# naver-ai/egtr

Hardware: AMD Instinct MI355X
Metric: images/sec end-to-end SGG, 600x1000 input, N=200 queries (higher is better)
Workload: dtype f32; 1 GPU; VG inference: ResNet-50, N=200, 6 enc/6 dec, 150 classes, 50 predicates, 600x1000, bs=1/GPU fp32 (BASELINE configs[1]); hip_graph=True, gemm_tuning=True, miopen_find=True, parallelism=replicas x1 (independent images, no collective)

## Files before the change

egtr_amd/csrc/ffn_x6.hip:

```cpp
#include <hip/hip_runtime.h>
#include <stdint.h>

#include "common.h"
#include "x6_common.h"
#include "xs_format.h"

namespace {
using namespace x6;

constexpr int kD = 256;
constexpr int kRows = 64;
constexpr int kKS = kD / 16;
constexpr int kFrag = xs::kFragBytes;
constexpr int kPanel = 2 * kKS * 2 * kFrag;
constexpr int kHbuf = 2 * 4 * 3 * kFrag;
constexpr int kStage = 24 * kFrag;
constexpr int kLds = kPanel + kHbuf + 3 * kStage;
static_assert(kLds == 160 * 1024, "the whole LDS of a CU");
constexpr int NL = 6;
typedef float f32x8 __attribute__((ext_vector_type(8)));

struct FfnArgs {
  const float* x;
  const float* res;
  const char* w1;
  const float* b1;
  const char* w2;
  const float* b2;
  const float* gamma;
  const float* beta;
  const float* pos;
  float* out;
  float* out_pos;
  int M, ldx, ldr, F, pos_rows;
  float eps;
  const char* wp;
  const float* bp;
  const float* gamma1;
  const float* beta1;
  float eps1;
};

__device__ __forceinline__ int swz(int x, int ks) { return x ^ (ks & 15) ^ ((x >> 5) << 2); }

__device__ __forceinline__ void build_panel(const float* __restrict__ x, int ldx, int M, int r0, int tid, int lane,
                                            char* panel, char* lo0, char* lo1) {
  float4 v[16];
#pragma unroll
  for (int it = 0; it < 16; ++it) {
    const int row = min(r0 + it * 4 + (tid >> 6), M - 1);
    v[it] = *reinterpret_cast<const float4*>(x + (size_t)row * ldx + 4 * lane);
  }
#pragma unroll
  for (int it = 0; it < 16; ++it) {
    const int row = it * 4 + (tid >> 6), rb = row >> 5, r = row & 31;
    const int ks = lane >> 2, off = (swz(r + 32 * ((lane >> 1) & 1), ks) << 4) + (lane & 1) * 8;
    const xs::Split3 s0 = xs::split3_fast(v[it].x), s1 = xs::split3_fast(v[it].y), s2 = xs::split3_fast(v[it].z),
                     s3 = xs::split3_fast(v[it].w);
    char* p = panel + ((rb * kKS + ks) * 2) * kFrag + off;
    *reinterpret_cast<uint2*>(p) = make_uint2(xs::pack_hi16(s0.hi, s1.hi), xs::pack_hi16(s2.hi, s3.hi));
    *reinterpret_cast<uint2*>(p + kFrag) = make_uint2(xs::pack_hi16(s0.mid, s1.mid), xs::pack_hi16(s2.mid, s3.mid));
    char* q = (rb == 0 ? lo0 : lo1) + ks * kFrag + off;
    *reinterpret_cast<uint2*>(q) = make_uint2(xs::pack_hi16(s0.lo, s1.lo), xs::pack_hi16(s2.lo, s3.lo));
  }
}

template <bool USE_RES_OF, class ResFn>
__device__ __forceinline__ void final_epilogue(const f32x16 (&acc2)[4], const FfnArgs& A, int r0, int wave, int lane,
                                               float* red, ResFn&& res_of) {
  const int wm = wave >> 1, wn = wave & 1, li = lane & 31, hf = lane >> 5;
  const int row = r0 + wm * 32 + li;
  float4 y[4][4];
#pragma unroll
  for (int t = 0; t < 4; ++t)
#pragma unroll
    for (int q = 0; q < 4; ++q) {
      const int col = (4 * wn + t) * 32 + 8 * q + 4 * hf;
      const float4 b = A.b2 != nullptr ? *reinterpret_cast<const float4*>(A.b2 + col) : make_float4(0.f, 0.f, 0.f, 0.f);
      y[t][q] = make_float4(acc2[t][4 * q + 0] + b.x, acc2[t][4 * q + 1] + b.y, acc2[t][4 * q + 2] + b.z,
                            acc2[t][4 * q + 3] + b.w);
    }
  if (A.gamma != nullptr) {
    const float* xr = A.res + (size_t)min(row, A.M - 1) * A.ldr;
#pragma unroll
    for (int t = 0; t < 4; ++t)
#pragma unroll
      for (int q = 0; q < 4; ++q) {
        float4 r;
        if constexpr (USE_RES_OF) r = res_of(t, q);
        else r = *reinterpret_cast<const float4*>(xr + (4 * wn + t) * 32 + 8 * q + 4 * hf);
        y[t][q].x += r.x; y[t][q].y += r.y; y[t][q].z += r.z; y[t][q].w += r.w;
      }
    __syncthreads();
    float sum = 0.f;
#pragma unroll
    for (int t = 0; t < 4; ++t)
#pragma unroll
      for (int q = 0; q < 4; ++q) sum += (y[t][q].x + y[t][q].y) + (y[t][q].z + y[t][q].w);
    sum += __shfl_xor(sum, 32);
    if (hf == 0) red[wave * 32 + li] = sum;
    __syncthreads();
    const float mean = (sum + red[(wave ^ 1) * 32 + li]) * (1.f / kD);
    float sq = 0.f;
#pragma unroll
    for (int t = 0; t < 4; ++t)
#pragma unroll
      for (int q = 0; q < 4; ++q) {
        y[t][q].x -= mean; y[t][q].y -= mean; y[t][q].z -= mean; y[t][q].w -= mean;
        sq += (y[t][q].x * y[t][q].x + y[t][q].y * y[t][q].y) + (y[t][q].z * y[t][q].z + y[t][q].w * y[t][q].w);
      }
    sq += __shfl_xor(sq, 32);
    if (hf == 0) red[128 + wave * 32 + li] = sq;
    __syncthreads();
    const float rstd = rsqrtf((sq + red[128 + (wave ^ 1) * 32 + li]) * (1.f / kD) + A.eps);
    const float* pr = A.out_pos != nullptr ? A.pos + (size_t)(min(row, A.M - 1) % A.pos_rows) * kD : nullptr;
#pragma unroll
    for (int t = 0; t < 4; ++t)
#pragma unroll
      for (int q = 0; q < 4; ++q) {
        const int col = (4 * wn + t) * 32 + 8 * q + 4 * hf;
        const float4 g = *reinterpret_cast<const float4*>(A.gamma + col), b = *reinterpret_cast<const float4*>(A.beta + col);
        y[t][q] = make_float4(y[t][q].x * rstd * g.x + b.x, y[t][q].y * rstd * g.y + b.y, y[t][q].z * rstd * g.z + b.z,
                              y[t][q].w * rstd * g.w + b.w);
        if (pr != nullptr && row < A.M) {
          const float4 p = *reinterpret_cast<const float4*>(pr + col);
          *reinterpret_cast<float4*>(A.out_pos + (size_t)row * kD + col) =
              make_float4(y[t][q].x + p.x, y[t][q].y + p.y, y[t][q].z + p.z, y[t][q].w + p.w);
        }
      }
  }
  if (row < A.M) {
#pragma unroll
    for (int t = 0; t < 4; ++t)
#pragma unroll
      for (int q = 0; q < 4; ++q)
        *reinterpret_cast<float4*>(A.out + (size_t)row * kD + (4 * wn + t) * 32 + 8 * q + 4 * hf) = y[t][q];
  }
}

__device__ __forceinline__ void layernorm_rows(float4 (&y)[4][4], const float* gamma, const float* beta, float eps, int wave,
                                               int lane, float* red) {
  const int wn = wave & 1, li = lane & 31, hf = lane >> 5;
  __syncthreads();
  float sum = 0.f;
#pragma unroll
  for (int t = 0; t < 4; ++t)
#pragma unroll
    for (int q = 0; q < 4; ++q) sum += (y[t][q].x + y[t][q].y) + (y[t][q].z + y[t][q].w);
  sum += __shfl_xor(sum, 32);
  if (hf == 0) red[wave * 32 + li] = sum;
  __syncthreads();
  const float mean = (sum + red[(wave ^ 1) * 32 + li]) * (1.f / kD);
  float sq = 0.f;
#pragma unroll
  for (int t = 0; t < 4; ++t)
#pragma unroll
    for (int q = 0; q < 4; ++q) {
      y[t][q].x -= mean; y[t][q].y -= mean; y[t][q].z -= mean; y[t][q].w -= mean;
      sq += (y[t][q].x * y[t][q].x + y[t][q].y * y[t][q].y) + (y[t][q].z * y[t][q].z + y[t][q].w * y[t][q].w);
    }
  sq += __shfl_xor(sq, 32);
  if (hf == 0) red[128 + wave * 32 + li] = sq;
  __syncthreads();
  const float rstd = rsqrtf((sq + red[128 + (wave ^ 1) * 32 + li]) * (1.f / kD) + eps);
#pragma unroll
  for (int t = 0; t < 4; ++t)
#pragma unroll
    for (int q = 0; q < 4; ++q) {
      const int col = (4 * wn + t) * 32 + 8 * q + 4 * hf;
      const float4 g = *reinterpret_cast<const float4*>(gamma + col), b = *reinterpret_cast<const float4*>(beta + col);
      y[t][q] = make_float4(y[t][q].x * rstd * g.x + b.x, y[t][q].y * rstd * g.y + b.y, y[t][q].z * rstd * g.z + b.z,
                            y[t][q].w * rstd * g.w + b.w);
    }
}

template <bool PROJ>
__global__ __launch_bounds__(256, 1) void ffn_x6_kernel(FfnArgs A) {
  extern __shared__ __attribute__((aligned(16))) char smem[];
  char* const panel = smem;
  char* const hbuf = smem + kPanel;
  char* const ring = smem + kPanel + kHbuf;
  const int tid = threadIdx.x, lane = tid & 63;
  const int wave = __builtin_amdgcn_readfirstlane(tid >> 6);
  const int wm = wave >> 1, wn = wave & 1;
  const int li = lane & 31, hf = lane >> 5;
  const unsigned lds_ring = (unsigned)reinterpret_cast<uintptr_t>((lds_char*)ring);
  const int r0 = blockIdx.x * kRows;
  const int nchunk = A.F >> 6, KSf = A.F >> 4;

  const unsigned voff = lane * 16;
  const int crot = blockIdx.x % nchunk;
  auto chunk_of = [&](int c) { const int t = c + crot; return t >= nchunk ? t - nchunk : t; };
  constexpr int NP = PROJ ? kKS : 0;
  const int nstages = NP + 8 * nchunk;
  const size_t nb_stride = (size_t)KSf * 3 * kFrag;
  auto stage_src = [&](int g, const char*& base, size_t& stride) {
    g = g < nstages ? g : nstages - 1;
    const bool pj = g < NP;
    const int gg = g - NP, c = chunk_of(pj ? 0 : gg >> 3), st = gg & 7;
    const bool l1 = st < 4;
    const char* b1 = A.w1 + ((size_t)((2 * c + (wave >> 1)) * kKS + 4 * (st & 3) + 2 * (wave & 1)) * 3) * kFrag;
    const char* b2 = A.w2 + ((size_t)(2 * wave * KSf + 4 * c + (st & 3)) * 3) * kFrag;
    base = l1 ? b1 : b2;
    stride = l1 ? (size_t)3 * kFrag : nb_stride;
    if constexpr (PROJ) {
      base = pj ? A.wp + ((size_t)(2 * wave * kKS + g) * 3) * kFrag : base;
      stride = pj ? (size_t)kKS * 3 * kFrag : stride;
    }
  };
  auto issue = [&](int g, int slot) {
    const unsigned dst = lds_ring + (unsigned)slot * kStage + (unsigned)wave * (NL * kFrag);
    const char* base;
    size_t stride;
    stage_src(g, base, stride);
#pragma unroll
    for (int i = 0; i < NL; ++i) dma16s(base + (i / 3) * stride + (i % 3) * kFrag, voff, dst + i * kFrag);
  };
  issue(0, 0);
  issue(1, 1);

  build_panel(A.x, A.ldx, A.M, r0, tid, lane, panel, hbuf, ring + 2 * kStage);
  __syncthreads();
  bf16x8 lo[kKS];
  {
    const char* q = (wm == 0 ? hbuf : ring + 2 * kStage);
#pragma unroll
    for (int ks = 0; ks < kKS; ++ks) lo[ks] = *reinterpret_cast<const bf16x8*>(q + ks * kFrag + (swz(lane, ks) << 4));
  }

  f32x16 acc2[4], acc1[2];
#pragma unroll
  for (int t = 0; t < 4; ++t)
#pragma unroll
    for (int r = 0; r < 16; ++r) acc2[t][r] = 0.f;

  auto pfrag = [&](int ks, int piece) {
    return *reinterpret_cast<const bf16x8*>(panel + ((wm * kKS + ks) * 2 + piece) * kFrag + (swz(lane, ks) << 4));
  };
  const char* const ph = hbuf + (wm * 4 * 3) * kFrag + lane * 16;
  const char* const pw = ring + (4 * wn * 3) * kFrag + lane * 16;
  auto frag = [](const char* p) { return *reinterpret_cast<const bf16x8*>(p); };

  auto stage = [&](auto S, const bf16x8 (&w)[4][3], bf16x8 (&wnx)[4][3], const bf16x8 (&a)[4][2], bf16x8 (&anx)[4][2], int g,
                   int slot_next, int slot_fill) {
    constexpr int s = decltype(S)::value;
    const char* const wn_src = pw + slot_next * kStage;
    const unsigned dst = lds_ring + (unsigned)slot_fill * kStage + (unsigned)wave * (NL * kFrag);
    const char* src;
    size_t sstride;
    stage_src(g + 3, src, sstride);
    static_for<24>([&](auto I) {
      constexpr int i = decltype(I)::value;
      constexpr int pwt[6] = {2, 0, 1, 1, 0, 0}, pat[6] = {0, 2, 1, 0, 1, 0};
      if constexpr (s < 4) {
        constexpr int pair = i / 12, term = (i % 12) / 2, par = i & 1, kl = 2 * pair + par;
        if constexpr (pat[term] == 2) acc1[par] = mfma(w[kl][pwt[term]], lo[4 * s + kl], acc1[par]);
        else acc1[par] = mfma(w[kl][pwt[term]], a[kl][pat[term]], acc1[par]);
        __builtin_amdgcn_sched_barrier(0);
      } else {
        constexpr int term = i / 4, t = i % 4;
        constexpr int ap = pat[term];
        acc2[t] = mfma(w[t][pwt[term]], a[ap >> 1][ap & 1], acc2[t]);
        __builtin_amdgcn_sched_barrier(0);
      }
      if constexpr ((i & 1) && (i >> 1) < NL) {
        constexpr int j = i >> 1;
        dma16s(src + (j / 3) * sstride + (j % 3) * kFrag, voff, dst + j * kFrag);
        __builtin_amdgcn_sched_barrier(0);
      }
      if constexpr (i >= 12 && i < 18) {
        constexpr int j = 2 * (i - 12);
        wnx[j / 3][j % 3] = frag(wn_src + j * kFrag);
        wnx[(j + 1) / 3][(j + 1) % 3] = frag(wn_src + (j + 1) * kFrag);
        __builtin_amdgcn_sched_barrier(0);
      }
      if constexpr (s < 8) {
        constexpr int sx = (s + 1) & 7;
        if constexpr (i >= 18 && i < 22 && sx < 4) {
          constexpr int kl = i - 18;
          anx[kl][0] = pfrag(4 * sx + kl, 0);
          anx[kl][1] = pfrag(4 * sx + kl, 1);
          __builtin_amdgcn_sched_barrier(0);
        }
        if constexpr (i == 18 && sx > 4) {
          anx[0][0] = frag(ph + ((sx - 4) * 3 + 0) * kFrag);
          anx[0][1] = frag(ph + ((sx - 4) * 3 + 1) * kFrag);
          anx[1][0] = frag(ph + ((sx - 4) * 3 + 2) * kFrag);
          __builtin_amdgcn_sched_barrier(0);
        }
      } else if constexpr (s - 8 + 1 < kKS) {
        if constexpr (i == 18) {
          anx[0][0] = pfrag(s - 8 + 1, 0);
          anx[0][1] = pfrag(s - 8 + 1, 1);
          anx[1][0] = lo[s - 8 + 1];
          __builtin_amdgcn_sched_barrier(0);
        }
      }
    });
  };

  bf16x8 w0[4][3], w1[4][3], a0[4][2], a1[4][2];
  f32x8 bias[4];
  wait_vm<NL>();
  wait_lgkm0();
  __builtin_amdgcn_s_barrier();
  issue(2, 2);
#pragma unroll
  for (int u = 0; u < 4; ++u)
#pragma unroll
    for (int p = 0; p < 3; ++p) w0[u][p] = frag(pw + (u * 3 + p) * kFrag);
  int slot = 0;
  int g = 0;
  auto stage_top = [&]() {
    wait_vm<NL>();
    wait_lgkm0();
    __builtin_amdgcn_s_barrier();
    __builtin_amdgcn_sched_barrier(0);
  };

  float4 y1[4][4];
  if constexpr (PROJ) {
    a0[0][0] = pfrag(0, 0);
    a0[0][1] = pfrag(0, 1);
    a0[1][0] = lo[0];
    static_for<kKS>([&](auto KS) {
      constexpr int ks = decltype(KS)::value;
      const int sn = slot == 2 ? 0 : slot + 1;
      stage_top();
      if constexpr ((ks & 1) == 0) stage(std::integral_constant<int, 8 + ks>{}, w0, w1, a0, a1, g, sn, slot);
      else stage(std::integral_constant<int, 8 + ks>{}, w1, w0, a1, a0, g, sn, slot);
      slot = sn;
      ++g;
    });
    const int row = r0 + wm * 32 + li;
    const float* xr = A.res + (size_t)min(row, A.M - 1) * A.ldr;
#pragma unroll
    for (int t = 0; t < 4; ++t)
#pragma unroll
      for (int q = 0; q < 4; ++q) {
        const int col = (4 * wn + t) * 32 + 8 * q + 4 * hf;
        const float4 b = *reinterpret_cast<const float4*>(A.bp + col), r = *reinterpret_cast<const float4*>(xr + col);
        y1[t][q] = make_float4(acc2[t][4 * q + 0] + b.x + r.x, acc2[t][4 * q + 1] + b.y + r.y, acc2[t][4 * q + 2] + b.z + r.z,
                               acc2[t][4 * q + 3] + b.w + r.w);
        acc2[t][4 * q + 0] = 0.f; acc2[t][4 * q + 1] = 0.f; acc2[t][4 * q + 2] = 0.f; acc2[t][4 * q + 3] = 0.f;
      }
    float* red = reinterpret_cast<float*>(hbuf + 16 * kFrag);
    layernorm_rows(y1, A.gamma1, A.beta1, A.eps1, wave, lane, red);
    uint2 plo[4][4];
#pragma unroll
    for (int t = 0; t < 4; ++t)
#pragma unroll
      for (int q = 0; q < 4; ++q) {
        const xs::Split3 s0 = xs::split3_fast(y1[t][q].x), s1 = xs::split3_fast(y1[t][q].y), s2 = xs::split3_fast(y1[t][q].z),
                         s3 = xs::split3_fast(y1[t][q].w);
        const int ks = 2 * (4 * wn + t) + (q >> 1);
        char* d = panel + ((wm * kKS + ks) * 2) * kFrag + (swz(li + 32 * (q & 1), ks) << 4) + 8 * hf;
        *reinterpret_cast<uint2*>(d) = make_uint2(xs::pack_hi16(s0.hi, s1.hi), xs::pack_hi16(s2.hi, s3.hi));
        *reinterpret_cast<uint2*>(d + kFrag) = make_uint2(xs::pack_hi16(s0.mid, s1.mid), xs::pack_hi16(s2.mid, s3.mid));
        plo[t][q] = make_uint2(xs::pack_hi16(s0.lo, s1.lo), xs::pack_hi16(s2.lo, s3.lo));
      }
#pragma unroll
    for (int rb = 0; rb < 2; ++rb) {
      if (wm == rb) {
#pragma unroll
        for (int t = 0; t < 4; ++t)
#pragma unroll
          for (int q = 0; q < 4; ++q) {
            const int ks = 2 * (4 * wn + t) + (q >> 1);
            *reinterpret_cast<uint2*>(hbuf + ks * kFrag + (swz(li + 32 * (q & 1), ks) << 4) + 8 * hf) = plo[t][q];
          }
      }
      __syncthreads();
      if (wm == rb) {
#pragma unroll
        for (int ks = 0; ks < kKS; ++ks) lo[ks] = *reinterpret_cast<const bf16x8*>(hbuf + ks * kFrag + (swz(lane, ks) << 4));
      }
      __syncthreads();
    }
  }
#pragma unroll
  for (int u = 0; u < 4; ++u) {
    a0[u][0] = pfrag(u, 0);
    a0[u][1] = pfrag(u, 1);
  }
#pragma unroll 1
  for (int c = 0; c < nchunk; ++c) {
    static_for<8>([&](auto S) {
      constexpr int s = decltype(S)::value;
      const int sn = slot == 2 ? 0 : slot + 1;
      stage_top();
      if constexpr (s == 4) {
        a0[0][0] = frag(ph + 0 * kFrag);
        a0[0][1] = frag(ph + 1 * kFrag);
        a0[1][0] = frag(ph + 2 * kFrag);
        __builtin_amdgcn_sched_barrier(0);
      }
      if constexpr (s == 0) {
#pragma unroll
        for (int t = 0; t < 2; ++t)
#pragma unroll
          for (int r = 0; r < 16; ++r) acc1[t][r] = 0.f;
        const float* bp = A.b1 + 64 * chunk_of(c) + 32 * wn;
        asm volatile("s_load_dwordx8 %0, %4, 0x0\n\ts_load_dwordx8 %1, %4, 0x20\n\ts_load_dwordx8 %2, %4, 0x40\n\t"
                     "s_load_dwordx8 %3, %4, 0x60"
                     : "=&s"(bias[0]), "=&s"(bias[1]), "=&s"(bias[2]), "=&s"(bias[3])
                     : "s"(bp));
      }
      if constexpr ((s & 1) == 0) stage(S, w0, w1, a0, a1, g, sn, slot);
      else stage(S, w1, w0, a1, a0, g, sn, slot);
      if constexpr (s == 3) {
        asm volatile("s_waitcnt lgkmcnt(0)" : "+s"(bias[0]), "+s"(bias[1]), "+s"(bias[2]), "+s"(bias[3]));
#pragma unroll
        for (int q = 0; q < 4; ++q) {
          float h[4];
#pragma unroll
          for (int j = 0; j < 4; ++j) {
            const float blo = bias[q][j], bhi = bias[q][4 + j];
            h[j] = egtr_relu(acc1[0][4 * q + j] + acc1[1][4 * q + j] + (hf ? bhi : blo));
          }
          char* dst = hbuf + ((wm * 4 + 2 * wn + (q >> 1)) * 3) * kFrag + (q & 1) * 512 + li * 16 + hf * 8;
          const xs::Split3 s0 = xs::split3_fast(h[0]), s1 = xs::split3_fast(h[1]), s2 = xs::split3_fast(h[2]),
                           s3 = xs::split3_fast(h[3]);
          *reinterpret_cast<uint2*>(dst) = make_uint2(xs::pack_hi16(s0.hi, s1.hi), xs::pack_hi16(s2.hi, s3.hi));
          *reinterpret_cast<uint2*>(dst + kFrag) = make_uint2(xs::pack_hi16(s0.mid, s1.mid), xs::pack_hi16(s2.mid, s3.mid));
          *reinterpret_cast<uint2*>(dst + 2 * kFrag) = make_uint2(xs::pack_hi16(s0.lo, s1.lo), xs::pack_hi16(s2.lo, s3.lo));
        }
      }
      slot = sn;
      ++g;
    });
  }
  wait_vm<0>();
  final_epilogue<PROJ>(acc2, A, r0, wave, lane, reinterpret_cast<float*>(ring), [&](int t, int q) { return y1[t][q]; });
  asm volatile("s_waitcnt vmcnt(0)" ::: "memory");
}


__global__ __launch_bounds__(256, 1) void proj_x6_kernel(FfnArgs A) {
  extern __shared__ __attribute__((aligned(16))) char smem[];
  char* const panel = smem;
  char* const ring = smem + kPanel;
  const int tid = threadIdx.x, lane = tid & 63;
  const int wave = __builtin_amdgcn_readfirstlane(tid >> 6);
  const int wm = wave >> 1, wn = wave & 1;
  const unsigned lds_ring = (unsigned)reinterpret_cast<uintptr_t>((lds_char*)ring);
  const int r0 = blockIdx.x * kRows;
  const unsigned voff = lane * 16;
  const int nw = A.F;
  auto src_of = [&](int w, int ks, int j) {
    if (ks >= kKS) { ks -= kKS; ++w; }
    if (w >= nw) { w = nw - 1; ks = kKS - 1; }
    return A.w2 + ((size_t)((8 * w + 2 * wave + j / 3) * kKS + ks) * 3 + j % 3) * kFrag;
  };
  auto issue = [&](int ks, int slot) {
    const unsigned dst = lds_ring + (unsigned)slot * kStage + (unsigned)wave * (NL * kFrag);
#pragma unroll
    for (int i = 0; i < NL; ++i) dma16s(src_of(0, ks, i), voff, dst + i * kFrag);
  };
  issue(0, 0);
  issue(1, 1);
  build_panel(A.x, A.ldx, A.M, r0, tid, lane, panel, ring + 2 * kStage, ring + 2 * kStage + kKS * kFrag);
  __syncthreads();
  bf16x8 lo[kKS];
  {
    const char* q = ring + 2 * kStage + wm * (kKS * kFrag);
#pragma unroll
    for (int ks = 0; ks < kKS; ++ks) lo[ks] = *reinterpret_cast<const bf16x8*>(q + ks * kFrag + (swz(lane, ks) << 4));
  }
  auto pfrag = [&](int ks, int piece) {
    return *reinterpret_cast<const bf16x8*>(panel + ((wm * kKS + ks) * 2 + piece) * kFrag + (swz(lane, ks) << 4));
  };
  const char* const pw = ring + (4 * wn * 3) * kFrag + lane * 16;
  auto frag = [](const char* p) { return *reinterpret_cast<const bf16x8*>(p); };
  bf16x8 w0[4][3], w1[4][3];
  wait_vm<NL>();
  wait_lgkm0();
  __builtin_amdgcn_s_barrier();
  issue(2, 2);
#pragma unroll
  for (int u = 0; u < 4; ++u)
#pragma unroll
    for (int p = 0; p < 3; ++p) w0[u][p] = frag(pw + (u * 3 + p) * kFrag);
  bf16x8 ahi = pfrag(0, 0), amid = pfrag(0, 1);
  int slot = 0;
#pragma unroll 1
  for (int w = 0; w < nw; ++w) {
    f32x16 acc2[4];
#pragma unroll
    for (int t = 0; t < 4; ++t)
#pragma unroll
      for (int r = 0; r < 16; ++r) acc2[t][r] = 0.f;
    static_for<kKS>([&](auto S) {
      constexpr int ks = decltype(S)::value;
      const int sn = slot == 2 ? 0 : slot + 1;
      wait_vm<NL>();
      wait_lgkm0();
      __builtin_amdgcn_s_barrier();
      __builtin_amdgcn_sched_barrier(0);
      const bf16x8 (&wc)[4][3] = (ks & 1) ? w1 : w0;
      bf16x8 (&wnx)[4][3] = (ks & 1) ? w0 : w1;
      const bf16x8 a0 = ahi, a1 = amid;
      const unsigned dst = lds_ring + (unsigned)slot * kStage + (unsigned)wave * (NL * kFrag);
      const char* const wn_src = pw + sn * kStage;
      static_for<24>([&](auto I) {
        constexpr int i = decltype(I)::value;
        constexpr int pwt[6] = {2, 0, 1, 1, 0, 0}, pat[6] = {0, 2, 1, 0, 1, 0};
        constexpr int term = i / 4, t = i % 4;
        if constexpr (pat[term] == 2) acc2[t] = mfma(wc[t][pwt[term]], lo[ks], acc2[t]);
        else acc2[t] = mfma(wc[t][pwt[term]], pat[term] == 0 ? a0 : a1, acc2[t]);
        __builtin_amdgcn_sched_barrier(0);
        if constexpr ((i & 1) && (i >> 1) < NL) {
          dma16s(src_of(w, ks + 3, i >> 1), voff, dst + (i >> 1) * kFrag);
          __builtin_amdgcn_sched_barrier(0);
        }
        if constexpr (i >= 12 && i < 18) {
          constexpr int j = 2 * (i - 12);
          wnx[j / 3][j % 3] = frag(wn_src + j * kFrag);
          wnx[(j + 1) / 3][(j + 1) % 3] = frag(wn_src + (j + 1) * kFrag);
          __builtin_amdgcn_sched_barrier(0);
        }
        if constexpr (i == 18) {
          ahi = pfrag((ks + 1) & (kKS - 1), 0);
          amid = pfrag((ks + 1) & (kKS - 1), 1);
          __builtin_amdgcn_sched_barrier(0);
        }
      });
      slot = sn;
    });
    FfnArgs Aw = A;
    Aw.out = A.out + (size_t)w * A.M * kD;
    Aw.b2 = A.b2 != nullptr ? A.b2 + w * kD : nullptr;
    if (w + 1 == nw) wait_vm<0>();
    final_epilogue<false>(acc2, Aw, r0, wave, lane, reinterpret_cast<float*>(ring), [](int, int) { return float4{}; });
  }
}

}

extern "C" int egtr_ffn_x6_f32(egtr_stream_t stream, const float* x, int ldx, const void* w1_xs, const float* b1,
                               const void* w2_xs, const float* b2, const float* ln_gamma, const float* ln_beta, float eps,
                               const float* pos, int pos_rows, float* out, float* out_pos, int M, int d_model, int ffn_dim) {
  if (!x || !w1_xs || !b1 || !w2_xs || !b2 || !out || M <= 0 || ldx < d_model) return EGTR_E_ARG;
  if ((ln_gamma == nullptr) != (ln_beta == nullptr) || (out_pos && (!pos || pos_rows <= 0 || !ln_gamma))) return EGTR_E_ARG;
  if (d_model != kD || ffn_dim <= 0 || ffn_dim % 64 || (ldx & 3) || (reinterpret_cast<uintptr_t>(x) & 15) ||
      (reinterpret_cast<uintptr_t>(out) & 15) || (reinterpret_cast<uintptr_t>(w1_xs) & 15) ||
      (reinterpret_cast<uintptr_t>(w2_xs) & 15) || (reinterpret_cast<uintptr_t>(b2) & 15) ||
      (out_pos && (reinterpret_cast<uintptr_t>(out_pos) & 15)) || (pos && (reinterpret_cast<uintptr_t>(pos) & 15)))
    return EGTR_E_UNSUPPORTED;
  static unsigned long long lds_raised = 0;
  if (int st = egtr_raise_dynamic_lds(reinterpret_cast<const void*>(ffn_x6_kernel<false>), kLds, &lds_raised)) return st;
  FfnArgs a{x, x, static_cast<const char*>(w1_xs), b1, static_cast<const char*>(w2_xs), b2, ln_gamma, ln_beta, pos, out,
            out_pos, M, ldx, ldx, ffn_dim, pos_rows, eps, nullptr, nullptr, nullptr, nullptr, 0.f};
  hipLaunchKernelGGL(ffn_x6_kernel<false>, dim3((M + kRows - 1) / kRows), dim3(256), kLds, static_cast<hipStream_t>(stream), a);
  return egtr_check_launch();
}

extern "C" int egtr_encoder_tail_x6_f32(egtr_stream_t stream, const float* context, int ldc, const float* hidden, int ldh,
                                        const void* wp_xs, const float* bp, const float* ln1_gamma, const float* ln1_beta,
                                        float eps1, const void* w1_xs, const float* b1, const void* w2_xs, const float* b2,
                                        const float* ln2_gamma, const float* ln2_beta, float eps2, const float* pos,
                                        int pos_rows, float* out, float* out_pos, int M, int d_model, int ffn_dim) {
  if (!context || !hidden || !wp_xs || !bp || !ln1_gamma || !ln1_beta || !w1_xs || !b1 || !w2_xs || !b2 || !ln2_gamma ||
      !ln2_beta || !out || M <= 0 || ldc < d_model || ldh < d_model)
    return EGTR_E_ARG;
  if (out_pos && (!pos || pos_rows <= 0)) return EGTR_E_ARG;
  if (d_model != kD || ffn_dim <= 0 || ffn_dim % 64 || (ldc & 3) || (ldh & 3)) return EGTR_E_UNSUPPORTED;
  for (const void* p : {(const void*)context, (const void*)hidden, wp_xs, (const void*)bp, (const void*)ln1_gamma,
                        (const void*)ln1_beta, w1_xs, w2_xs, (const void*)b2, (const void*)ln2_gamma, (const void*)ln2_beta,
                        (const void*)out, (const void*)out_pos, (const void*)pos})
    if (reinterpret_cast<uintptr_t>(p) & 15) return EGTR_E_UNSUPPORTED;
  static unsigned long long lds_raised = 0;
  if (int st = egtr_raise_dynamic_lds(reinterpret_cast<const void*>(ffn_x6_kernel<true>), kLds, &lds_raised)) return st;
  FfnArgs a{context, hidden, static_cast<const char*>(w1_xs), b1, static_cast<const char*>(w2_xs), b2, ln2_gamma, ln2_beta,
            pos, out, out_pos, M, ldc, ldh, ffn_dim, pos_rows, eps2, static_cast<const char*>(wp_xs), bp, ln1_gamma,
            ln1_beta, eps1};
  hipLaunchKernelGGL(ffn_x6_kernel<true>, dim3((M + kRows - 1) / kRows), dim3(256), kLds, static_cast<hipStream_t>(stream), a);
  return egtr_check_launch();
}

extern "C" int egtr_proj_ln_x6_f32(egtr_stream_t stream, const float* x, int ldx, const void* w_xs, const float* bias,
                                   const float* residual, int ldr, const float* ln_gamma, const float* ln_beta, float eps,
                                   const float* pos, int pos_rows, float* out, float* out_pos, int M, int d_model) {
  if (!x || !w_xs || !bias || !out || M <= 0 || ldx < d_model) return EGTR_E_ARG;
  if ((ln_gamma == nullptr) != (ln_beta == nullptr) || (ln_gamma && (!residual || ldr < d_model)) ||
      (out_pos && (!pos || pos_rows <= 0 || !ln_gamma)))
    return EGTR_E_ARG;
  if (d_model != kD || (ldx & 3) || (ldr & 3) || (reinterpret_cast<uintptr_t>(x) & 15) ||
      (reinterpret_cast<uintptr_t>(out) & 15) || (reinterpret_cast<uintptr_t>(w_xs) & 15) ||
      (reinterpret_cast<uintptr_t>(bias) & 15) || (reinterpret_cast<uintptr_t>(residual) & 15) ||
      (out_pos && (reinterpret_cast<uintptr_t>(out_pos) & 15)) || (pos && (reinterpret_cast<uintptr_t>(pos) & 15)))
    return EGTR_E_UNSUPPORTED;
  constexpr int lds = kPanel + 3 * kStage + 8 * kFrag;
  static unsigned long long lds_raised = 0;
  if (int st = egtr_raise_dynamic_lds(reinterpret_cast<const void*>(proj_x6_kernel), lds, &lds_raised)) return st;
  FfnArgs a{x, residual, nullptr, nullptr, static_cast<const char*>(w_xs), bias, ln_gamma, ln_beta, pos, out, out_pos,
            M, ldx, ldr, 1, pos_rows, eps};
  hipLaunchKernelGGL(proj_x6_kernel, dim3((M + kRows - 1) / kRows), dim3(256), lds, static_cast<hipStream_t>(stream), a);
  return egtr_check_launch();
}

extern "C" int egtr_proj_multi_x6_f32(egtr_stream_t stream, const float* x, int ldx, const void* w_xs, const float* bias,
                                      float* out, int M, int d_model, int num_weights) {
  if (!x || !w_xs || !out || M <= 0 || ldx < d_model || num_weights <= 0) return EGTR_E_ARG;
  if (d_model != kD || (ldx & 3) || (reinterpret_cast<uintptr_t>(x) & 15) || (reinterpret_cast<uintptr_t>(out) & 15) ||
      (reinterpret_cast<uintptr_t>(w_xs) & 15) || (bias && (reinterpret_cast<uintptr_t>(bias) & 15)))
    return EGTR_E_UNSUPPORTED;
  constexpr int lds = kPanel + 3 * kStage + 8 * kFrag;
  static unsigned long long lds_raised = 0;
  if (int st = egtr_raise_dynamic_lds(reinterpret_cast<const void*>(proj_x6_kernel), lds, &lds_raised)) return st;
  FfnArgs a{x, nullptr, nullptr, nullptr, static_cast<const char*>(w_xs), bias, nullptr, nullptr, nullptr, out, nullptr,
            M, ldx, 0, num_weights, 0, 0.f};
  hipLaunchKernelGGL(proj_x6_kernel, dim3((M + kRows - 1) / kRows), dim3(256), lds, static_cast<hipStream_t>(stream), a);
  return egtr_check_launch();
}
```

Before: 395.9 images/sec.

## Software-pipeline FFN hidden epilogue into next chunk's layer-2 stages

Restructures the FFN chunk loop so the ReLU/bias/split3/pack/store of the hidden activations for chunk c is spread across the layer-2 MFMA stages of the following chunk instead of running as a serial block after stage 3. The stage order is rotated (prologue of four layer-1 stages, steady-state loop, epilogue of four layer-2 stages), so the DMA source address generator is rewritten branch-free and computed incrementally one stage ahead. The epilogue args are also reloaded from the kernarg segment to ease register pressure. It adds optional s_memtime instrumentation behind a macro, and it risks scheduling/register pressure from interleaving and ordering mistakes in the hidden-buffer handoff.

```diff
diff --git a/egtr_amd/csrc/ffn_x6.hip b/egtr_amd/csrc/ffn_x6.hip
--- a/egtr_amd/csrc/ffn_x6.hip
+++ b/egtr_amd/csrc/ffn_x6.hip
@@ -1,4 +1,5 @@
 #include <hip/hip_runtime.h>
+#include <stddef.h>
 #include <stdint.h>
 
 #include "common.h"
@@ -19,6 +20,19 @@
 static_assert(kLds == 160 * 1024, "the whole LDS of a CU");
 constexpr int NL = 6;
 typedef float f32x8 __attribute__((ext_vector_type(8)));
+
+#ifdef EGTR_FFN_X6_TIMING
+constexpr int kRecWg = 256, kRecN = 24;
+__device__ unsigned g_ffn_x6_rec[kRecWg][kRecN];
+#define FFN_T(v)                                        \
+  do {                                                  \
+    __builtin_amdgcn_sched_barrier(0);                  \
+    (v) = (unsigned)__builtin_amdgcn_s_memtime();       \
+    __builtin_amdgcn_sched_barrier(0);                  \
+  } while (0)
+#else
+#define FFN_T(v) do { } while (0)
+#endif
 
 struct FfnArgs {
   const float* x;
@@ -187,6 +201,10 @@
   const unsigned lds_ring = (unsigned)reinterpret_cast<uintptr_t>((lds_char*)ring);
   const int r0 = blockIdx.x * kRows;
   const int nchunk = A.F >> 6, KSf = A.F >> 4;
+#ifdef EGTR_FFN_X6_TIMING
+  unsigned tk0, tl0, ts[8], th = 0, te = 0, tsum[6] = {0, 0, 0, 0, 0, 0};
+  FFN_T(tk0);
+#endif
 
   const unsigned voff = lane * 16;
   const int crot = blockIdx.x % nchunk;
@@ -196,9 +214,11 @@
   const size_t nb_stride = (size_t)KSf * 3 * kFrag;
   auto stage_src = [&](int g, const char*& base, size_t& stride) {
     g = g < nstages ? g : nstages - 1;
-    const bool pj = g < NP;
-    const int gg = g - NP, c = chunk_of(pj ? 0 : gg >> 3), st = gg & 7;
-    const bool l1 = st < 4;
+    const int gg = g - NP, h = gg - 4, q = h >> 3;
+    const int pji = (int)((unsigned)gg >> 31), first = (int)((unsigned)h >> 31);
+    const int l1i = first | (((~h >> 2) & 1) & (int)((unsigned)(q - (nchunk - 1)) >> 31));
+    const bool pj = pji != 0, l1 = l1i != 0;
+    const int c = chunk_of((q + l1i) & (first - 1)), st = gg & 3;
     const char* b1 = A.w1 + ((size_t)((2 * c + (wave >> 1)) * kKS + 4 * (st & 3) + 2 * (wave & 1)) * 3) * kFrag;
     const char* b2 = A.w2 + ((size_t)(2 * wave * KSf + 4 * c + (st & 3)) * 3) * kFrag;
     base = l1 ? b1 : b2;
@@ -208,6 +228,8 @@
       stride = pj ? (size_t)kKS * 3 * kFrag : stride;
     }
   };
+  const char* fsrc;
+  unsigned fstride;
   auto issue = [&](int g, int slot) {
     const unsigned dst = lds_ring + (unsigned)slot * kStage + (unsigned)wave * (NL * kFrag);
     const char* base;
@@ -241,14 +263,50 @@
   const char* const pw = ring + (4 * wn * 3) * kFrag + lane * 16;
   auto frag = [](const char* p) { return *reinterpret_cast<const bf16x8*>(p); };
 
-  auto stage = [&](auto S, const bf16x8 (&w)[4][3], bf16x8 (&wnx)[4][3], const bf16x8 (&a)[4][2], bf16x8 (&anx)[4][2], int g,
-                   int slot_next, int slot_fill) {
+  f32x8 bias[4];
+  xs::Split3 hsp[2];
+  uint2 hpk[4][3];
+  float hv[6];
+  auto ho_value_a = [&](auto E) {
+    constexpr int e = decltype(E)::value, q = e >> 2, j = e & 3;
+    const float blo = bias[q][j], bhi = bias[q][4 + j];
+    float& v = hv[e % 6];
+    v = egtr_relu(acc1[0][4 * q + j] + acc1[1][4 * q + j] + (hf ? bhi : blo));
+    asm volatile("" : "+v"(v));
+  };
+  auto ho_value_b = [&](auto E) {
+    constexpr int e = decltype(E)::value;
+    xs::Split3& v = hsp[e & 1];
+    v = xs::split3_fast(hv[e % 6]);
+    asm volatile("" : "+v"(v.hi), "+v"(v.mid), "+v"(v.lo));
+  };
+  auto ho_value = [&](auto E) {
+    ho_value_a(E);
+    ho_value_b(E);
+  };
+  auto ho_pack = [&](auto P) {
+    constexpr int p = decltype(P)::value, q = p >> 1;
+    unsigned h = xs::pack_hi16(hsp[0].hi, hsp[1].hi), m = xs::pack_hi16(hsp[0].mid, hsp[1].mid),
+                   l = xs::pack_hi16(hsp[0].lo, hsp[1].lo);
+    asm volatile("" : "+v"(h), "+v"(m), "+v"(l));
+    if constexpr ((p & 1) == 0) { hpk[q][0].x = h; hpk[q][1].x = m; hpk[q][2].x = l; }
+    else { hpk[q][0].y = h; hpk[q][1].y = m; hpk[q][2].y = l; }
+  };
+  auto ho_store = [&](auto N) {
+    constexpr int n = decltype(N)::value, q = n / 3, piece = n % 3;
+    char* dst = hbuf + ((wm * 4 + 2 * wn + (q >> 1)) * 3 + piece) * kFrag + (q & 1) * 512 + li * 16 + hf * 8;
+    *reinterpret_cast<uint2*>(dst) = hpk[q][piece];
+  };
+
+  auto stage = [&](auto S, auto HOc, const bf16x8 (&w)[4][3], bf16x8 (&wnx)[4][3], const bf16x8 (&a)[4][2],
+                   bf16x8 (&anx)[4][2], int g, int slot_next, int slot_fill) {
     constexpr int s = decltype(S)::value;
+    constexpr bool HO = decltype(HOc)::value != 0;
     const char* const wn_src = pw + slot_next * kStage;
     const unsigned dst = lds_ring + (unsigned)slot_fill * kStage + (unsigned)wave * (NL * kFrag);
-    const char* src;
-    size_t sstride;
-    stage_src(g + 3, src, sstride);
+    const char* const src = fsrc;
+    const size_t sstride = fstride;
+    size_t stride64;
     static_for<24>([&](auto I) {
       constexpr int i = decltype(I)::value;
       constexpr int pwt[6] = {2, 0, 1, 1, 0, 0}, pat[6] = {0, 2, 1, 0, 1, 0};
@@ -268,6 +326,30 @@
         dma16s(src + (j / 3) * sstride + (j % 3) * kFrag, voff, dst + j * kFrag);
         __builtin_amdgcn_sched_barrier(0);
       }
+      if constexpr (HO && s >= 4 && s < 7) {
+        constexpr int e0 = 6 * (s - 4);
+        constexpr int kb[10] = {0, 1, -1, 2, 3, -2, -9, 4, 5, -3};
+        if constexpr (i < 12 && (i & 1) == 0 && e0 + (i >> 1) < 16) {
+          ho_value_a(std::integral_constant<int, e0 + (i >> 1)>{});
+          __builtin_amdgcn_sched_barrier(0);
+        }
+        if constexpr (i >= 12 && i < 22) {
+          constexpr int k = kb[i - 12];
+          if constexpr (k >= 0 && e0 + k < 16) {
+            ho_value_b(std::integral_constant<int, e0 + k>{});
+            __builtin_amdgcn_sched_barrier(0);
+          }
+          if constexpr (k < 0 && k > -9 && e0 + 2 * (-k - 1) < 16) {
+            ho_pack(std::integral_constant<int, e0 / 2 + (-k - 1)>{});
+            __builtin_amdgcn_sched_barrier(0);
+          }
+        }
+      }
+      if constexpr (HO && s == 7 && i < 12 && (i & 1) == 0) {
+        ho_store(std::integral_constant<int, i>{});
+        ho_store(std::integral_constant<int, i + 1>{});
+        __builtin_amdgcn_sched_barrier(0);
+      }
       if constexpr (i >= 12 && i < 18) {
         constexpr int j = 2 * (i - 12);
         wnx[j / 3][j % 3] = frag(wn_src + j * kFrag);
@@ -276,13 +358,15 @@
       }
       if constexpr (s < 8) {
         constexpr int sx = (s + 1) & 7;
-        if constexpr (i >= 18 && i < 22 && sx < 4) {
+        constexpr bool nx_l1 = sx < 4 || (s == 3 && !HO);
+        constexpr bool nx_l2 = sx > 4 || (s == 3 && HO);
+        if constexpr (i >= 18 && i < 22 && nx_l1) {
           constexpr int kl = i - 18;
-          anx[kl][0] = pfrag(4 * sx + kl, 0);
-          anx[kl][1] = pfrag(4 * sx + kl, 1);
+          anx[kl][0] = pfrag(4 * (sx & 3) + kl, 0);
+          anx[kl][1] = pfrag(4 * (sx & 3) + kl, 1);
           __builtin_amdgcn_sched_barrier(0);
         }
-        if constexpr (i == 18 && sx > 4) {
+        if constexpr (i == 18 && nx_l2) {
           anx[0][0] = frag(ph + ((sx - 4) * 3 + 0) * kFrag);
           anx[0][1] = frag(ph + ((sx - 4) * 3 + 1) * kFrag);
           anx[1][0] = frag(ph + ((sx - 4) * 3 + 2) * kFrag);
@@ -296,11 +380,20 @@
           __builtin_amdgcn_sched_barrier(0);
         }
       }
+      if constexpr (i == 22) {
+        if constexpr ((s & 3) == 0) {
+          stage_src(min(g + 4, nstages - 4), fsrc, stride64);
+          fstride = (unsigned)stride64;
+        } else {
+          fsrc += fstride == 3u * kFrag ? 12 * kFrag : 3 * kFrag;
+        }
+        asm volatile("" : "+s"(fsrc), "+s"(fstride));
+        __builtin_amdgcn_sched_barrier(0);
+      }
     });
   };
 
   bf16x8 w0[4][3], w1[4][3], a0[4][2], a1[4][2];
-  f32x8 bias[4];
   wait_vm<NL>();
   wait_lgkm0();
   __builtin_amdgcn_s_barrier();
@@ -309,6 +402,11 @@
   for (int u = 0; u < 4; ++u)
 #pragma unroll
     for (int p = 0; p < 3; ++p) w0[u][p] = frag(pw + (u * 3 + p) * kFrag);
+  {
+    size_t stride64;
+    stage_src(3, fsrc, stride64);
+    fstride = (unsigned)stride64;
+  }
   int slot = 0;
   int g = 0;
   auto stage_top = [&]() {
@@ -327,8 +425,8 @@
       constexpr int ks = decltype(KS)::value;
       const int sn = slot == 2 ? 0 : slot + 1;
       stage_top();
-      if constexpr ((ks & 1) == 0) stage(std::integral_constant<int, 8 + ks>{}, w0, w1, a0, a1, g, sn, slot);
-      else stage(std::integral_constant<int, 8 + ks>{}, w1, w0, a1, a0, g, sn, slot);
+      if constexpr ((ks & 1) == 0) stage(std::integral_constant<int, 8 + ks>{}, std::integral_constant<int, 0>{}, w0, w1, a0, a1, g, sn, slot);
+      else stage(std::integral_constant<int, 8 + ks>{}, std::integral_constant<int, 0>{}, w1, w0, a1, a0, g, sn, slot);
       slot = sn;
       ++g;
     });
@@ -383,56 +481,108 @@
     a0[u][0] = pfrag(u, 0);
     a0[u][1] = pfrag(u, 1);
   }
+  auto walk_stage = [&](auto S, auto HOc, int cb) {
+    constexpr int s = decltype(S)::value;
+    constexpr bool HO = decltype(HOc)::value != 0;
+    const int sn = slot == 2 ? 0 : slot + 1;
+#ifdef EGTR_FFN_X6_TIMING
+    if constexpr (HO && (s == 0 || s == 4 || s == 7)) FFN_T(ts[s]);
+    if constexpr (!HO && (s == 4 || s == 5)) FFN_T(ts[s]);
+#endif
+    stage_top();
+    if constexpr (s == 4 && !HO) {
+      a0[0][0] = frag(ph + 0 * kFrag);
+      a0[0][1] = frag(ph + 1 * kFrag);
+      a0[1][0] = frag(ph + 2 * kFrag);
+      __builtin_amdgcn_sched_barrier(0);
+    }
+    if constexpr (s == 0) {
+#pragma unroll
+      for (int t = 0; t < 2; ++t)
+#pragma unroll
+        for (int r = 0; r < 16; ++r) acc1[t][r] = 0.f;
+      const float* bp = A.b1 + 64 * chunk_of(cb) + 32 * wn;
+      asm volatile("s_load_dwordx8 %0, %4, 0x0\n\ts_load_dwordx8 %1, %4, 0x20\n\ts_load_dwordx8 %2, %4, 0x40\n\t"
+                   "s_load_dwordx8 %3, %4, 0x60"
+                   : "=&s"(bias[0]), "=&s"(bias[1]), "=&s"(bias[2]), "=&s"(bias[3])
+                   : "s"(bp));
+    }
+    if constexpr (s == 4 && HO)
+      asm volatile("s_waitcnt lgkmcnt(0)" : "+s"(bias[0]), "+s"(bias[1]), "+s"(bias[2]), "+s"(bias[3]));
+    if constexpr ((s & 1) == 0) stage(S, HOc, w0, w1, a0, a1, g, sn, slot);
+    else stage(S, HOc, w1, w0, a1, a0, g, sn, slot);
+    slot = sn;
+    ++g;
+  };
+  constexpr std::integral_constant<int, 0> kPlain{};
+  constexpr std::integral_constant<int, 1> kSteady{};
+#ifdef EGTR_FFN_X6_TIMING
+  FFN_T(tl0);
+#endif
+  static_for<4>([&](auto S) { walk_stage(S, kPlain, 0); });
+#ifdef EGTR_FFN_X6_TIMING
+  FFN_T(th);
+#endif
+  asm volatile("s_waitcnt lgkmcnt(0)" : "+s"(bias[0]), "+s"(bias[1]), "+s"(bias[2]), "+s"(bias[3]));
+  static_for<16>([&](auto E) {
+    ho_value(E);
+    if constexpr (decltype(E)::value & 1) ho_pack(std::integral_constant<int, (decltype(E)::value >> 1)>{});
+  });
+  static_for<12>([&](auto N) { ho_store(N); });
+#ifdef EGTR_FFN_X6_TIMING
+  FFN_T(te);
+  tsum[4] = te - th;
+#endif
 #pragma unroll 1
-  for (int c = 0; c < nchunk; ++c) {
-    static_for<8>([&](auto S) {
-      constexpr int s = decltype(S)::value;
-      const int sn = slot == 2 ? 0 : slot + 1;
-      stage_top();
-      if constexpr (s == 4) {
-        a0[0][0] = frag(ph + 0 * kFrag);
-        a0[0][1] = frag(ph + 1 * kFrag);
-        a0[1][0] = frag(ph + 2 * kFrag);
-        __builtin_amdgcn_sched_barrier(0);
-      }
-      if constexpr (s == 0) {
-#pragma unroll
-        for (int t = 0; t < 2; ++t)
-#pragma unroll
-          for (int r = 0; r < 16; ++r) acc1[t][r] = 0.f;
-        const float* bp = A.b1 + 64 * chunk_of(c) + 32 * wn;
-        asm volatile("s_load_dwordx8 %0, %4, 0x0\n\ts_load_dwordx8 %1, %4, 0x20\n\ts_load_dwordx8 %2, %4, 0x40\n\t"
-                     "s_load_dwordx8 %3, %4, 0x60"
-                     : "=&s"(bias[0]), "=&s"(bias[1]), "=&s"(bias[2]), "=&s"(bias[3])
-                     : "s"(bp));
-      }
-      if constexpr ((s & 1) == 0) stage(S, w0, w1, a0, a1, g, sn, slot);
-      else stage(S, w1, w0, a1, a0, g, sn, slot);
-      if constexpr (s == 3) {
-        asm volatile("s_waitcnt lgkmcnt(0)" : "+s"(bias[0]), "+s"(bias[1]), "+s"(bias[2]), "+s"(bias[3]));
-#pragma unroll
-        for (int q = 0; q < 4; ++q) {
-          float h[4];
-#pragma unroll
-          for (int j = 0; j < 4; ++j) {
-            const float blo = bias[q][j], bhi = bias[q][4 + j];
-            h[j] = egtr_relu(acc1[0][4 * q + j] + acc1[1][4 * q + j] + (hf ? bhi : blo));
-          }
-          char* dst = hbuf + ((wm * 4 + 2 * wn + (q >> 1)) * 3) * kFrag + (q & 1) * 512 + li * 16 + hf * 8;
-          const xs::Split3 s0 = xs::split3_fast(h[0]), s1 = xs::split3_fast(h[1]), s2 = xs::split3_fast(h[2]),
-                           s3 = xs::split3_fast(h[3]);
-          *reinterpret_cast<uint2*>(dst) = make_uint2(xs::pack_hi16(s0.hi, s1.hi), xs::pack_hi16(s2.hi, s3.hi));
-          *reinterpret_cast<uint2*>(dst + kFrag) = make_uint2(xs::pack_hi16(s0.mid, s1.mid), xs::pack_hi16(s2.mid, s3.mid));
-          *reinterpret_cast<uint2*>(dst + 2 * kFrag) = make_uint2(xs::pack_hi16(s0.lo, s1.lo), xs::pack_hi16(s2.lo, s3.lo));
-        }
-      }
-      slot = sn;
-      ++g;
-    });
-  }
+  for (int c = 0; c + 1 < nchunk; ++c) {
+    static_for<8>([&](auto S) { walk_stage(S, kSteady, c + 1); });
+#ifdef EGTR_FFN_X6_TIMING
+    FFN_T(te);
+    tsum[0] += ts[4] - ts[0];
+    tsum[2] += ts[7] - ts[4];
+    tsum[3] += te - ts[7];
+#endif
+  }
+  static_for<4>([&](auto S) { walk_stage(std::integral_constant<int, 4 + decltype(S)::value>{}, kPlain, 0); });
+#ifdef EGTR_FFN_X6_TIMING
+  unsigned tl1;
+  FFN_T(tl1);
+#endif
   wait_vm<0>();
-  final_epilogue<PROJ>(acc2, A, r0, wave, lane, reinterpret_cast<float*>(ring), [&](int t, int q) { return y1[t][q]; });
+#if defined(__HIP_DEVICE_COMPILE__)
+  typedef const __attribute__((address_space(4))) unsigned* KernargWords;
+  KernargWords ka = (KernargWords)__builtin_amdgcn_kernarg_segment_ptr();
+  asm volatile("" : "+s"(ka));
+  FfnArgs Ae;
+  static_assert(sizeof(FfnArgs) % 4 == 0, "copied in 32-bit words");
+#pragma unroll
+  for (unsigned i = 0; i < sizeof(FfnArgs) / 4; ++i) reinterpret_cast<unsigned*>(&Ae)[i] = ka[i];
+  auto global_ptr = [&](size_t offset) {
+    typedef const __attribute__((address_space(4))) unsigned long long* KernargQuads;
+    const unsigned long long bits = *(KernargQuads)((const __attribute__((address_space(4))) char*)ka + offset);
+    return (float*)(__attribute__((address_space(1))) float*)bits;
+  };
+  Ae.res = global_ptr(offsetof(FfnArgs, res)); Ae.b2 = global_ptr(offsetof(FfnArgs, b2));
+  Ae.gamma = global_ptr(offsetof(FfnArgs, gamma)); Ae.beta = global_ptr(offsetof(FfnArgs, beta));
+  Ae.pos = global_ptr(offsetof(FfnArgs, pos)); Ae.out = global_ptr(offsetof(FfnArgs, out));
+  Ae.out_pos = global_ptr(offsetof(FfnArgs, out_pos));
+#else
+  const FfnArgs& Ae = A;
+#endif
+  final_epilogue<PROJ>(acc2, Ae, r0, wave, lane, reinterpret_cast<float*>(ring), [&](int t, int q) { return y1[t][q]; });
   asm volatile("s_waitcnt vmcnt(0)" ::: "memory");
+#ifdef EGTR_FFN_X6_TIMING
+  unsigned tk1;
+  FFN_T(tk1);
+  if (tid == 0 && blockIdx.x < kRecWg) {
+    unsigned* rec = g_ffn_x6_rec[blockIdx.x];
+    for (int k = 0; k < 5; ++k) rec[k] = tsum[k];
+    rec[5] = ts[5] - ts[4];
+    rec[6] = tl1 - tl0;
+    rec[7] = tk1 - tk0;
+    rec[8] = tl0 - tk0;
+  }
+#endif
 }
 
 
@@ -537,6 +687,13 @@
 
 }
 
+#ifdef EGTR_FFN_X6_TIMING
+extern "C" int egtr_ffn_x6_stamps(unsigned* host_out) {
+  return hipMemcpyFromSymbol(host_out, HIP_SYMBOL(g_ffn_x6_rec), sizeof(unsigned) * kRecWg * kRecN) == hipSuccess ? EGTR_OK
+                                                                                                                  : EGTR_E_LAUNCH;
+}
+#endif
+
 extern "C" int egtr_ffn_x6_f32(egtr_stream_t stream, const float* x, int ldx, const void* w1_xs, const float* b1,
                                const void* w2_xs, const float* b2, const float* ln_gamma, const float* ln_beta, float eps,
                                const float* pos, int pos_rows, float* out, float* out_pos, int M, int d_model, int ffn_dim) {
```

New measurement: 402.2 images/sec, median of 6. 1.02x the previous value.
